# psy-ex/svt-av1-psy

Measured on AMD Instinct MI355X. Metric: Mblocks/s per kernel (SAD, FwdTxfm2d, CDEF) + encoder fps @1080p preset 8, higher is better.
Workload: dtype u8

## Files before the change

svt-av1-psy_amd/csrc/sad.hip:

```cpp
#include "svt_hip_common.h"
#include "../../include/svtav1_hip.h"
#include "hme_geom.h"
#include <vector>

namespace {

struct __attribute__((packed, aligned(4))) U64A4 { unsigned long long v; };
struct __attribute__((aligned(4))) u32x4_a4 { uint32_t x, y, z, w; };
struct __attribute__((aligned(16))) u32x4_a16 { uint32_t x, y, z, w; };

constexpr uint32_t MAX_SAD_VALUE = 128 * 128 * 255;
constexpr int      ME_TW         = 64;
constexpr int      ME_TH         = 32;
constexpr int      KEY_POS_BITS  = 11;
constexpr uint32_t ME_WAVE_MAX_W = 24, ME_WAVE_MAX_H = 16;

__device__ __forceinline__ void stage_rows_u8(uint32_t* lds, int pitch_dw, const uint8_t* g, uint32_t gstride, int width,
                                              int rows, int tid, int nthreads) {
    const int total = rows * pitch_dw;
    for (int i = tid; i < total; i += nthreads) {
        const int r   = i / pitch_dw;
        const int k   = i - r * pitch_dw;
        const int col = k * 4;
        uint32_t  v   = 0;
// ... 115 lines not shown
__device__ __forceinline__ uint32_t dpp_add_quad_xor2(uint32_t v) {
    return v + (uint32_t)__builtin_amdgcn_update_dpp(0, (int)v, 0x4E, 0xf, 0xf, false);
}
__device__ __forceinline__ uint32_t dpp_add_row_ror4(uint32_t v) {
    return v + (uint32_t)__builtin_amdgcn_update_dpp(0, (int)v, 0x124, 0xf, 0xf, false);
}
__device__ __forceinline__ uint32_t dpp_add_row_ror8(uint32_t v) {
    return v + (uint32_t)__builtin_amdgcn_update_dpp(0, (int)v, 0x128, 0xf, 0xf, false);
}
__device__ __forceinline__ uint32_t umin32(uint32_t a, uint32_t b) { return a < b ? a : b; }


constexpr int ME_PITCH = 34;

__device__ __forceinline__ uint32_t dpp_scatter_sum_quads(const uint32_t (&v)[4]) {
#ifdef SVT_HIP_EMU
    const uint32_t a0 = dpp_add_row_ror8(v[0]), a1 = dpp_add_row_ror8(v[1]), a2 = dpp_add_row_ror8(v[2]), a3 = dpp_add_row_ror8(v[3]);
    const uint32_t t0 = (uint32_t)__builtin_amdgcn_update_dpp((int)a0, (int)a2, 0xE4, 0xf, 0xc, false);
    const uint32_t t1 = (uint32_t)__builtin_amdgcn_update_dpp((int)a1, (int)a3, 0xE4, 0xf, 0xc, false);
    const uint32_t y  = (uint32_t)__builtin_amdgcn_update_dpp((int)t0, (int)t1, 0xE4, 0xf, 0xa, false);
    const uint32_t x  = y + (uint32_t)__builtin_amdgcn_update_dpp(0, (int)t0, 0x12C, 0xf, 0x5, false);
    return x + (uint32_t)__builtin_amdgcn_update_dpp(0, (int)t1, 0x124, 0xf, 0xa, false);
#else
    uint32_t t0, t1;
    asm("s_nop 1\n\t"
        "v_add_u32_dpp %0, %2, %2 row_ror:8 row_mask:0xf bank_mask:0x3\n\t"
        "v_add_u32_dpp %0, %4, %4 row_ror:8 row_mask:0xf bank_mask:0xc\n\t"
        "v_add_u32_dpp %1, %3, %3 row_ror:8 row_mask:0xf bank_mask:0x3\n\t"
        "v_add_u32_dpp %1, %5, %5 row_ror:8 row_mask:0xf bank_mask:0xc\n\t"
        "v_add_u32_dpp %0, %0, %0 row_ror:12 row_mask:0xf bank_mask:0x5\n\t"
        "s_nop 0\n\t"
        "v_add_u32_dpp %0, %1, %1 row_ror:4 row_mask:0xf bank_mask:0xa"
        : "=&v"(t0), "=&v"(t1)
        : "v"(v[0]), "v"(v[1]), "v"(v[2]), "v"(v[3]));
    return t0;
#endif
}

constexpr int ME_WAVE_QSUM_DW = 32;
__device__ __forceinline__ void me_lds_order() {
    __builtin_amdgcn_fence(__ATOMIC_ACQ_REL, "wavefront");
    __builtin_amdgcn_wave_barrier();
}
__device__ __forceinline__ uint32_t sum_rows_pair(const uint32_t a, const uint32_t b) {
#ifdef SVT_HIP_EMU
    const int l = (int)(threadIdx.x & 63);
    uint32_t  t = 0;
    for (int r = 0; r < 4; r++) {
        const uint32_t ar = (uint32_t)__shfl((int)a, (l & 15) + 16 * r), br = (uint32_t)__shfl((int)b, (l & 15) + 16 * r);
        t += ((l >> 4) & 1) ? br : ar;
    }
    return t;
#else
    const auto     x16 = __builtin_amdgcn_permlane16_swap(a, b, false, false);
    const uint32_t two = x16[0] + x16[1];
    const auto     x32 = __builtin_amdgcn_permlane32_swap(two, two, false, false);
    return x32[0] + x32[1];
#endif
}
template <bool SUB, bool FULL, int PITCH = ME_PITCH, bool QLDS = false>
__device__ __forceinline__ void me_search_strips(const uint32_t* __restrict__ win, const uint32_t (&s)[8][2], int Wt, int Ht, int g0, int gstep, int l,
                                                 uint32_t& best8, uint32_t& best16, uint32_t& best32, uint32_t& best64, unsigned long long* qsum = nullptr) {
    const int bx = (l & 1) | ((l >> 1) & 2) | ((l >> 2) & 4);
    const int by = ((l >> 1) & 1) | ((l >> 2) & 2) | ((l >> 3) & 4);
    const int q  = l & 3, c = (l >> 2) & 3;
    unsigned long long* const qslot = QLDS ? qsum + (l >> 2) : nullptr;
    const uint16_t* const     qmine = QLDS ? (const uint16_t*)qslot + q : nullptr;
    const int      G    = (Wt + 3) >> 2;
    const uint32_t qsel = 0x0c0c0100u + 0x0202u * (uint32_t)q;
    uint32_t       himask = 0xffff0000u;
    SVT_HIP_OPAQUE_I32(himask);
    constexpr uint32_t NO_STEP = 0x1ffffu;
    uint32_t       b16 = 0xffffffffu, b32 = 0xffffffffu, b64 = 0xffffffffu;
    constexpr bool PAIRG = QLDS && !SUB;
    uint32_t       b64s  = 0xffffffffu;
    constexpr uint32_t NO_SUM = 0x7ffffu;
    uint32_t       p32 = NO_SUM, b32p = 0xffffffffu, b64p = 0xffffffffu;
    int            kc = 0;
    for (int g = g0; g < G; g += gstep) {
        const uint32_t* colp   = win + (by * 8) * PITCH + bx * 2 + g;
        const int       nvalid = (Wt - 4 * g) < 4 ? (Wt - 4 * g) : 4;
        const uint32_t inv1 = nvalid > 1 ? 0u : 0xffffffffu, inv2 = nvalid > 2 ? 0u : 0xffffffffu, inv3 = nvalid > 3 ? 0u : 0xffffffffu;
        const uint32_t invq = q < nvalid ? 0u : 0xffffffffu;
        auto track16 = [&](const uint32_t sad16, const uint32_t at) {
            const uint32_t k16 = (sad16 << KEY_POS_BITS) | at;
            b16 = umin32(b16, FULL ? k16 : (k16 | invq));
        };
        auto track16x2 = [&](const uint32_t sad16a, const uint32_t sad16b, const uint32_t at) {
            const uint32_t ka = (sad16a << KEY_POS_BITS) | at, kb = (sad16b << KEY_POS_BITS) | (at + ME_TW);
            b16 = FULL ? umin32(umin32(b16, ka), kb) : umin32(b16, umin32(ka, kb) | invq);
        };
        U64A4 ra[8], rb[8];
#pragma unroll
        for (int r = 0; r < 7; r++) {
            ra[r] = *(const U64A4*)(colp + r * PITCH);
            rb[r] = *(const U64A4*)(colp + r * PITCH + 1);
        }
        uint32_t pos = (uint32_t)(4 * g);
        uint32_t v0  = 0;
        uint32_t s32a = 0;
        for (int yb = 0; yb < Ht; yb += 8) {
            const uint32_t* rowp = colp + (yb + 7) * PITCH;
#pragma unroll
            for (int h = 0; h < 2; h++) {
                if (yb + 4 * h < Ht) {
                    uint32_t v[4] = {NO_STEP, NO_STEP, NO_STEP, NO_STEP};
#pragma unroll
                    for (int j = 0; j < 4; j++) {
                        const int i = 4 * h + j;
                        if (yb + i < Ht) {
                            ra[(i + 7) & 7] = *(const U64A4*)(rowp + i * PITCH);
                            rb[(i + 7) & 7] = *(const U64A4*)(rowp + i * PITCH + 1);
                            unsigned long long acc = 0;
#pragma unroll
                            for (int r = 0; r < 8; r += (SUB ? 2 : 1)) {
                                acc = __builtin_amdgcn_qsad_pk_u16_u8(ra[(i + r) & 7].v, s[r][0], acc);
                                acc = __builtin_amdgcn_qsad_pk_u16_u8(rb[(i + r) & 7].v, s[r][1], acc);
                            }
                            if (SUB) acc <<= 1;
                            const uint32_t lo = (uint32_t)acc, hi = (uint32_t)(acc >> 32);
                            const uint32_t p1 = FULL ? pos + 1 : ((pos + 1) | inv1), p2 = FULL ? pos + 2 : ((pos + 2) | inv2), p3 = FULL ? pos + 3 : ((pos + 3) | inv3);
                            const uint32_t k0 = (lo << 16) | pos, k1 = (lo & himask) | p1, k2 = (hi << 16) | p2, k3 = (hi & himask) | p3;
                            best8 = umin32(umin32(best8, k0), k1);
                            best8 = umin32(umin32(best8, k2), k3);
                            if (QLDS) {
                                me_lds_order();
                                *qslot = 0ull;
                                me_lds_order();
                                atomicAdd(qslot, acc);
                                me_lds_order();
                                v[j] = *qmine;
                                if (PAIRG) {
                                    if (j == 2) track16x2(v[0], v[1], pos - 2 * ME_TW);
                                } else if (j > 0) {
                                    track16(v[j - 1], pos - ME_TW);
                                }
                            } else {
                                const uint32_t tlo = dpp_add_quad_xor2(dpp_add_quad_xor1(lo));
                                const uint32_t thi = dpp_add_quad_xor2(dpp_add_quad_xor1(hi));
                                v[j] = __builtin_amdgcn_perm(thi, tlo, qsel);
                                track16(v[j], pos);
                            }
                            pos += ME_TW;
                        }
                    }
                    if (PAIRG) {
                        const int left = Ht - (yb + 4 * h);
                        if (left >= 4) {
                            asm volatile("");
                            track16x2(v[2], v[3], pos - 2 * ME_TW);
                        } else if (left == 3) {
                            asm volatile("");
                            track16(v[2], pos - ME_TW);
                        } else if (left == 2) {
                            asm volatile("");
                            track16x2(v[0], v[1], pos - 2 * ME_TW);
                        } else {
                            track16(v[0], pos - ME_TW);
                        }
                    } else if (QLDS) {
                        const int left = Ht - (yb + 4 * h);
                        track16(left >= 4 ? v[3] : (left == 3 ? v[2] : (left == 2 ? v[1] : v[0])), pos - ME_TW);
                    }
                    v0 = v[0];
                    if (PAIRG) {
                        const int      left   = Ht - (yb + 4 * h);
                        const bool     paired = left >= 6 - 4 * h;
                        const uint32_t gposa  = (uint32_t)(4 * g + ME_TW * yb);
                        if (h == 0 && left >= 2) {
                            s32a = dpp_scatter_sum_quads(v);
                            if (!paired) {
                                const uint32_t k32 = (s32a << KEY_POS_BITS) | gposa;
                                b32 = umin32(b32, FULL ? k32 : (k32 | invq));
                                const uint32_t k64 = (sum_rows_pair(s32a, s32a) << KEY_POS_BITS) | gposa;
                                b64s = umin32(b64s, FULL ? k64 : (k64 | invq));
                            }
                        }
                        if (h == 1 && paired) {
                            const uint32_t s32b = dpp_scatter_sum_quads(v);
                            const uint32_t k32a = (s32a << KEY_POS_BITS) | gposa, k32b = (s32b << KEY_POS_BITS) | (gposa + 4 * ME_TW);
                            b32 = FULL ? umin32(umin32(b32, k32a), k32b) : umin32(b32, umin32(k32a, k32b) | invq);
                            const uint32_t k64 = (sum_rows_pair(s32a, s32b) << KEY_POS_BITS) | gposa;
                            b64 = umin32(b64, FULL ? k64 : (k64 | invq));
                        }
                    } else if (yb + 4 * h + 1 < Ht) {
                        const uint32_t gpos  = (uint32_t)(4 * g + ME_TW * (yb + 4 * h));
                        const uint32_t sad32 = dpp_scatter_sum_quads(v);
                        const uint32_t k32   = (sad32 << KEY_POS_BITS) | gpos;
                        b32 = umin32(b32, FULL ? k32 : (k32 | invq));
                        const auto     x16   = __builtin_amdgcn_permlane16_swap(sad32, sad32, false, false);
                        const uint32_t pair  = x16[0] + x16[1];
                        const auto     x32   = __builtin_amdgcn_permlane32_swap(pair, pair, false, false);
                        const uint32_t sad64 = x32[0] + x32[1];
                        const uint32_t k64   = (sad64 << KEY_POS_BITS) | gpos;
                        b64 = umin32(b64, FULL ? k64 : (k64 | invq));
                    }
                }
            }
        }
        if ((Ht & 3) == 1) {
            const uint32_t sum = dpp_add_row_ror4(dpp_add_row_ror8(v0));
            if (c == kc && (FULL || q < nvalid)) p32 = sum;
            if (++kc == 4 || g + gstep >= G) {
                const uint32_t gpos  = (uint32_t)(4 * (g - (kc - 1) * gstep) + ME_TW * (Ht - 1));
                b32p = umin32(b32p, (p32 << KEY_POS_BITS) | gpos);
                const auto     x16   = __builtin_amdgcn_permlane16_swap(p32, p32, false, false);
                const uint32_t pair  = x16[0] + x16[1];
                const auto     x32   = __builtin_amdgcn_permlane32_swap(pair, pair, false, false);
                const uint32_t sad64 = x32[0] + x32[1];
                b64p = umin32(b64p, (sad64 << KEY_POS_BITS) | gpos);
                p32 = NO_SUM;
                kc  = 0;
            }
        }
    }
    best16 = umin32(best16, b16 | (uint32_t)q);
    best32 = umin32(best32, b32 | (uint32_t)(q | (c << 6)));
    best64 = umin32(best64, b64 | (uint32_t)(q | (c << 6) | (PAIRG ? ((l << 4) & 256) : 0)));
    if (PAIRG) best64 = umin32(best64, b64s | (uint32_t)(q | (c << 6)));
    best32 = umin32(best32, b32p | (uint32_t)(q | (4 * gstep * c)));
    best64 = umin32(best64, b64p | (uint32_t)(q | (4 * gstep * c)));
}

template <bool SUB>
__global__ __launch_bounds__(256, 4) void me_fullpel_kernel(const uint8_t* __restrict__ src_base, const uint8_t* __restrict__ ref_base,
                                                         const SvtHipMeSearchDesc* __restrict__ descs, uint32_t n,
                                                         uint32_t tiles_x,
                                                         uint32_t* __restrict__ best_sad, uint32_t* __restrict__ best_mv,
                                                         unsigned long long* __restrict__ keys) {
    HIP_DYNAMIC_SHARED(uint32_t, smem)
    uint32_t* src_lds  = smem;
    uint32_t* best_lds = smem + 64 * 16;
    uint32_t* win      = smem + 64 * 16 + 88;

    const int      tid  = threadIdx.x;
    const uint32_t item = xcd_remap(blockIdx.x, n);
    const uint32_t tile = blockIdx.y;
    const SvtHipMeSearchDesc d = descs[item];
    const int W   = d.search_area_width, H = d.search_area_height;
    const int tx0 = (int)(tile % tiles_x) * ME_TW;
    const int ty0 = (int)(tile / tiles_x) * ME_TH;
    if (tx0 >= W || ty0 >= H) {
        if (tile == 0 && keys == nullptr && tid < SVT_HIP_ME_NUM_BLOCKS) {
            best_sad[(size_t)item * SVT_HIP_ME_NUM_BLOCKS + tid] = MAX_SAD_VALUE;
            best_mv[(size_t)item * SVT_HIP_ME_NUM_BLOCKS + tid]  = 0;
        }
        return;
    }
    const int Wt = (W - tx0) < ME_TW ? (W - tx0) : ME_TW;
    const int Ht = (H - ty0) < ME_TH ? (H - ty0) : ME_TH;

    {
        uint32_t vs[1][4], vw[3][4];
        stage_rows_load<1, 2>(vs, src_base + d.src_off, d.src_stride, 64, 64, tid);
        stage_rows_load<3, 3>(vw, ref_base + d.ref_off + (size_t)ty0 * d.ref_stride + tx0, d.ref_stride, 64 + Wt - 1, 64 + Ht - 1, tid);
        stage_rows_store<1, 2>(vs, src_lds, 16, 64, tid);
        stage_rows_store<3, 3>(vw, win, ME_PITCH, 64 + Ht - 1, tid);
    }
    if (tid < 88) best_lds[tid] = 0xffffffffu;
    __syncthreads();

    const int l  = tid & 63;
    const int wv = tid >> 6;
    uint32_t s[8][2];
    {
        const int bx = (l & 1) | ((l >> 1) & 2) | ((l >> 2) & 4);
        const int by = ((l >> 1) & 1) | ((l >> 2) & 2) | ((l >> 3) & 4);
#pragma unroll
        for (int r = 0; r < 8; r++) {
            s[r][0] = src_lds[(by * 8 + r) * 16 + bx * 2 + 0];
            s[r][1] = src_lds[(by * 8 + r) * 16 + bx * 2 + 1];
        }
    }
    uint32_t best8 = 0xffffffffu, best16 = 0xffffffffu, best32 = 0xffffffffu, best64 = 0xffffffffu;
    if ((Wt & 3) == 0) me_search_strips<SUB, true>(win, s, Wt, Ht, wv, 4, l, best8, best16, best32, best64);
    else me_search_strips<SUB, false>(win, s, Wt, Ht, wv, 4, l, best8, best16, best32, best64);

    atomicMin(&best_lds[21 + l], best8);
    atomicMin(&best_lds[5 + (l >> 2)], best16);
    atomicMin(&best_lds[1 + (l >> 4)], best32);
    atomicMin(&best_lds[0], best64);
    __syncthreads();
    if (tid < SVT_HIP_ME_NUM_BLOCKS) {
        const uint32_t key = best_lds[tid];
        const uint32_t sad = tid >= 21 ? (key >> 16) : (key >> KEY_POS_BITS);
        const int      X   = tx0 + (int)(key & 63u);
        const int      Y   = ty0 + (int)((key >> 6) & 31u);
        const size_t   o   = (size_t)item * SVT_HIP_ME_NUM_BLOCKS + tid;
        if (keys == nullptr) {
            best_sad[o] = sad;
            best_mv[o]  = ((uint32_t)(uint16_t)(Y + d.y_search_area_origin) << 16) | (uint16_t)(X + d.x_search_area_origin);
        } else {
            atomicMin(&keys[o], ((unsigned long long)sad << 32) | (unsigned long long)(uint32_t)(Y * W + X));
        }
    }
}

struct __attribute__((packed, aligned(1))) u32x2_a1 { uint32_t x, y; };
__device__ __forceinline__ uint32_t dpp_min_quad_xor1(uint32_t v) { return umin32(v, (uint32_t)__builtin_amdgcn_update_dpp(-1, (int)v, 0xB1, 0xf, 0xf, false)); }
__device__ __forceinline__ uint32_t dpp_min_quad_xor2(uint32_t v) { return umin32(v, (uint32_t)__builtin_amdgcn_update_dpp(-1, (int)v, 0x4E, 0xf, 0xf, false)); }
__device__ __forceinline__ uint32_t dpp_min_row_ror4(uint32_t v) { return umin32(v, (uint32_t)__builtin_amdgcn_update_dpp(-1, (int)v, 0x124, 0xf, 0xf, false)); }
__device__ __forceinline__ uint32_t dpp_min_row_ror8(uint32_t v) { return umin32(v, (uint32_t)__builtin_amdgcn_update_dpp(-1, (int)v, 0x128, 0xf, 0xf, false)); }

template <int NF, int PITCH>
__device__ __forceinline__ void stage_window_wave(uint32_t* lds, const uint8_t* g, const uint32_t gstride, const int width, const int rows, const int l) {
    constexpr int RPI = 64 / NF;
    const int     rem = width & 15, back = 16 - rem;
    const bool    p0 = rem != 0 && l < rows, p1 = rem != 0 && l + 64 < rows;
    u32x4_a1      t[2] = {{0u, 0u, 0u, 0u}, {0u, 0u, 0u, 0u}};
    const uint32_t tail_off = (uint32_t)l * gstride + (uint32_t)(width - 16);
    if (p0) t[0] = *(const u32x4_a1*)(g + tail_off);
    if (p1) t[1] = *(const u32x4_a1*)(g + (size_t)64 * gstride + tail_off);

    const int lr = l / NF, lc = l - lr * NF;
    if (lr < RPI) {
        const uint32_t goff = (uint32_t)lr * gstride + (uint32_t)lc * 16u;
        uint32_t*      lp   = lds + lr * PITCH + lc * 4;
        for (int r0 = 0; r0 < rows; r0 += 4 * RPI) {
            const uint8_t* gb = g + (size_t)r0 * gstride;
            u32x4_a1       v[4];
#pragma unroll
            for (int k = 0; k < 4; k++)
                if (r0 + k * RPI + lr < rows) v[k] = *(const u32x4_a1*)(gb + (size_t)(k * RPI) * gstride + goff);
#pragma unroll
            for (int k = 0; k < 4; k++)
                if (r0 + k * RPI + lr < rows) {
                    uint32_t* o = lp + (r0 + k * RPI) * PITCH;
                    *(u32x2_a8*)(o + 0) = u32x2_a8{v[k].x, v[k].y};
                    *(u32x2_a8*)(o + 2) = u32x2_a8{v[k].z, v[k].w};
                }
        }
    }
#pragma unroll
    for (int k = 0; k < 2; k++)
        if (k == 0 ? p0 : p1) {
            uint32_t x0 = t[k].x, x1 = t[k].y, x2 = t[k].z, x3 = t[k].w;
            if (back & 4) { x0 = x1; x1 = x2; x2 = x3; x3 = 0; }
            if (back & 8) { x0 = x2; x1 = x3; x2 = 0; x3 = 0; }
            const uint32_t bs = (uint32_t)back & 3u;
            x0 = __builtin_amdgcn_alignbyte(x1, x0, bs);
            x1 = __builtin_amdgcn_alignbyte(x2, x1, bs);
            x2 = __builtin_amdgcn_alignbyte(x3, x2, bs);
            x3 = __builtin_amdgcn_alignbyte(0u, x3, bs);
            uint32_t* o = lds + (l + 64 * k) * PITCH + NF * 4;
            if (NF * 4 + 0 < PITCH) *(u32x2_a8*)(o + 0) = u32x2_a8{x0, x1};
            if (NF * 4 + 2 < PITCH) *(u32x2_a8*)(o + 2) = u32x2_a8{x2, x3};
        }
}

template <bool SUB, int PITCH>
__global__ __launch_bounds__(256) void me_fullpel_wave_kernel(const uint8_t* __restrict__ src_base, const uint8_t* __restrict__ ref_base,
                                                              const SvtHipMeSearchDesc* __restrict__ descs, const uint32_t n, const int win_dw,
                                                              uint32_t* __restrict__ best_sad, uint32_t* __restrict__ best_mv) {
    HIP_DYNAMIC_SHARED(uint32_t, smem)
    const int      l    = threadIdx.x & 63, wv = __builtin_amdgcn_readfirstlane((int)(threadIdx.x >> 6));
    const uint32_t item = xcd_remap(blockIdx.x, gridDim.x) * 4 + (uint32_t)wv;
    if (item >= n) return;
    const SvtHipMeSearchDesc d = descs[item];
    const int    W = d.search_area_width, H = d.search_area_height;
    const size_t o = (size_t)item * SVT_HIP_ME_NUM_BLOCKS;
    if (W <= 0 || H <= 0) {
        for (int k = l; k < SVT_HIP_ME_NUM_BLOCKS; k += 64) { best_sad[o + k] = MAX_SAD_VALUE; best_mv[o + k] = 0; }
        return;
    }
    uint32_t* win = smem + wv * (win_dw + ME_WAVE_QSUM_DW);
    const int bx = (l & 1) | ((l >> 1) & 2) | ((l >> 2) & 4);
    const int by = ((l >> 1) & 1) | ((l >> 2) & 2) | ((l >> 3) & 4);
    uint32_t  s[8][2];
    {
        const uint8_t* sp = src_base + d.src_off + (size_t)(by * 8) * d.src_stride + bx * 8;
#pragma unroll
        for (int r = 0; r < 8; r++) {
            const u32x2_a1 t = *(const u32x2_a1*)(sp + (size_t)r * d.src_stride);
            s[r][0] = t.x; s[r][1] = t.y;
        }
    }
    const int width = 64 + W - 1;
    if (PITCH >= 22 && (width >> 4) == 5) stage_window_wave<5, PITCH>(win, ref_base + d.ref_off, d.ref_stride, width, 64 + H - 1, l);
    else stage_window_wave<4, PITCH>(win, ref_base + d.ref_off, d.ref_stride, width, 64 + H - 1, l);
    __builtin_amdgcn_wave_barrier();

    uint32_t best8 = 0xffffffffu, best16 = 0xffffffffu, best32 = 0xffffffffu, best64 = 0xffffffffu;
    if ((W & 3) == 0) me_search_strips<SUB, true, PITCH, true>(win, s, W, H, 0, 1, l, best8, best16, best32, best64, (unsigned long long*)(win + win_dw));
    else me_search_strips<SUB, false, PITCH, true>(win, s, W, H, 0, 1, l, best8, best16, best32, best64, (unsigned long long*)(win + win_dw));
    best16 = dpp_min_quad_xor2(dpp_min_quad_xor1(best16));
    best32 = dpp_min_row_ror8(dpp_min_row_ror4(dpp_min_quad_xor2(dpp_min_quad_xor1(best32))));
    best64 = dpp_min_row_ror8(dpp_min_row_ror4(dpp_min_quad_xor2(dpp_min_quad_xor1(best64))));
    {
        const auto x16 = __builtin_amdgcn_permlane16_swap(best64, best64, false, false);
        best64         = umin32(x16[0], x16[1]);
        const auto x32 = __builtin_amdgcn_permlane32_swap(best64, best64, false, false);
        best64         = umin32(x32[0], x32[1]);
    }
    const int xo = d.x_search_area_origin, yo = d.y_search_area_origin;
    auto emit = [&](const int idx, const uint32_t key, const bool is8) {
        const uint32_t sad = is8 ? (key >> 16) : (key >> KEY_POS_BITS);
        const int      X = (int)(key & 63u), Y = (int)((key >> 6) & 31u);
        best_sad[o + idx] = sad;
        best_mv[o + idx]  = ((uint32_t)(uint16_t)(Y + yo) << 16) | (uint16_t)(X + xo);
    };
    emit(21 + l, best8, true);
    const int      q    = l & 3;
    const uint32_t mine = q == 1 ? best16 : (q == 2 ? best32 : best64);
    const int      r32  = 64 * l - 56, r16 = 16 * l - 76;
    const uint32_t key  = (uint32_t)__builtin_amdgcn_ds_bpermute(l < 5 ? (r32 > 0 ? r32 : 0) : r16, (int)mine);
    if (l < 21) emit(l, key, false);
}

__global__ void me_finalize_kernel(const SvtHipMeSearchDesc* __restrict__ descs, uint32_t n, const unsigned long long* __restrict__ keys,
                                   uint32_t* __restrict__ best_sad, uint32_t* __restrict__ best_mv) {
    const uint32_t i = blockIdx.x * blockDim.x + threadIdx.x;
    if (i >= n * SVT_HIP_ME_NUM_BLOCKS) return;
    const SvtHipMeSearchDesc d   = descs[i / SVT_HIP_ME_NUM_BLOCKS];
    const unsigned long long key = keys[i];
    if (key == ~0ull) {
        best_sad[i] = MAX_SAD_VALUE;
        best_mv[i]  = 0;
        return;
    }
    const uint32_t pos = (uint32_t)key;
    const int      W   = d.search_area_width;
    const int      X = (int)(pos % (uint32_t)W), Y = (int)(pos / (uint32_t)W);
    best_sad[i]        = (uint32_t)(key >> 32);
    best_mv[i]         = ((uint32_t)(uint16_t)(Y + d.y_search_area_origin) << 16) | (uint16_t)(X + d.x_search_area_origin);
}

__device__ __forceinline__ uint32_t wave_sum(uint32_t v) {
    v += (uint32_t)__shfl_xor((int)v, 32);
    v += (uint32_t)__shfl_xor((int)v, 16);
    v = dpp_add_row_ror8(v);
    v = dpp_add_row_ror4(v);
    v = dpp_add_quad_xor2(v);
    v = dpp_add_quad_xor1(v);
    return v;
}

template <int CHUNK>
__device__ __forceinline__ uint32_t sad_chunks(const uint8_t* __restrict__ src, const uint8_t* __restrict__ ref, uint32_t ss, uint32_t rs,
                                               int cpr, int cshift, int total, int l) {
    uint32_t sad = 0;
    for (int i0 = l; i0 < total; i0 += 256) {
        uint32_t av[4][CHUNK / 4], bv[4][CHUNK / 4];
#pragma unroll
        for (int k = 0; k < 4; ++k) {
            const int  i  = i0 + 64 * k;
            const bool in = i < total;
            const int  r  = cshift >= 0 ? (i >> cshift) : (i / cpr);
            const int  c  = i - r * cpr;
            const uint8_t* pa = src + (size_t)r * ss + c * CHUNK;
            const uint8_t* pb = ref + (size_t)r * rs + c * CHUNK;
            if (CHUNK == 16) {
                u32x4_a1 a = {0, 0, 0, 0}, b = {0, 0, 0, 0};
                if (in) { a = *(const u32x4_a1*)pa; b = *(const u32x4_a1*)pb; }
                av[k][0] = a.x; av[k][CHUNK / 4 > 1 ? 1 : 0] = a.y; av[k][CHUNK / 4 > 2 ? 2 : 0] = a.z; av[k][CHUNK / 4 > 3 ? 3 : 0] = a.w;
                bv[k][0] = b.x; bv[k][CHUNK / 4 > 1 ? 1 : 0] = b.y; bv[k][CHUNK / 4 > 2 ? 2 : 0] = b.z; bv[k][CHUNK / 4 > 3 ? 3 : 0] = b.w;
            } else {
                u32_a1 a = {0}, b = {0};
                if (in) { a = *(const u32_a1*)pa; b = *(const u32_a1*)pb; }
                av[k][0] = a.x; bv[k][0] = b.x;
            }
        }
#pragma unroll
        for (int k = 0; k < 4; ++k)
#pragma unroll
            for (int j = 0; j < CHUNK / 4; ++j) sad = __builtin_amdgcn_sad_u8(av[k][j], bv[k][j], sad);
    }
    return sad;
}

__global__ __launch_bounds__(256) void sad_nxm_kernel(const uint8_t* __restrict__ src_base, const uint8_t* __restrict__ ref_base,
                                                      const SvtHipSadPair* __restrict__ pairs, uint32_t n, int width, int height,
                                                      uint32_t* __restrict__ sad_out) {
    const int      l    = threadIdx.x & 63;
    const uint32_t pair = xcd_remap(blockIdx.x, gridDim.x) * 4 + (threadIdx.x >> 6);
    if (pair >= n) return;
    const SvtHipSadPair p   = pairs[pair];
    const uint8_t*      src = src_base + p.src_off;
    const uint8_t*      ref = ref_base + p.ref_off;
    uint32_t            sad = 0;
    if ((width & 15) == 0) {
        const int cpr = width >> 4;
        sad = sad_chunks<16>(src, ref, p.src_stride, p.ref_stride, cpr, (cpr & (cpr - 1)) ? -1 : __builtin_ctz(cpr), cpr * height, l);
    } else if ((width & 3) == 0) {
        const int cpr = width >> 2;
        sad = sad_chunks<4>(src, ref, p.src_stride, p.ref_stride, cpr, (cpr & (cpr - 1)) ? -1 : __builtin_ctz(cpr), cpr * height, l);
    } else {
        const int total = width * height;
        for (int i = l; i < total; i += 64) {
            const int r = i / width, c = i - r * width;
            const int a = src[(size_t)r * p.src_stride + c], b = ref[(size_t)r * p.ref_stride + c];
            sad += (uint32_t)(a > b ? a - b : b - a);
        }
    }
    sad = wave_sum(sad);
    if (l == 0) sad_out[pair] = sad;
}

constexpr int SADP_PPW = 4;
struct SadRegs { uint32_t a[4][4], b[4][4]; };
__device__ __forceinline__ void sadp_issue(SadRegs& r, const uint8_t* __restrict__ src, const uint8_t* __restrict__ ref, const SvtHipSadPair& p, const int cpr,
                                           const int cshift, const int total, const int l) {
#pragma unroll
    for (int k = 0; k < 4; ++k) {
        const int  i  = l + 64 * k;
        const bool in = i < total;
        const int  rr = i >> cshift, c = i - (rr << cshift);
        u32x4_a1 a = {0, 0, 0, 0}, b = {0, 0, 0, 0};
        if (in) {
            a = *(const u32x4_a1*)(src + p.src_off + (size_t)rr * p.src_stride + c * 16);
            b = *(const u32x4_a1*)(ref + p.ref_off + (size_t)rr * p.ref_stride + c * 16);
        }
        r.a[k][0] = a.x; r.a[k][1] = a.y; r.a[k][2] = a.z; r.a[k][3] = a.w;
        r.b[k][0] = b.x; r.b[k][1] = b.y; r.b[k][2] = b.z; r.b[k][3] = b.w;
    }
}
__device__ __forceinline__ uint32_t sadp_reduce(const SadRegs& r) {
    uint32_t sad = 0;
#pragma unroll
    for (int k = 0; k < 4; ++k)
#pragma unroll
        for (int j = 0; j < 4; ++j) sad = __builtin_amdgcn_sad_u8(r.a[k][j], r.b[k][j], sad);
    return wave_sum(sad);
}
__global__ __launch_bounds__(256) void sad_nxm_pipe_kernel(const uint8_t* __restrict__ src_base, const uint8_t* __restrict__ ref_base,
                                                           const SvtHipSadPair* __restrict__ pairs, uint32_t n, int cshift , int total,
                                                           uint32_t* __restrict__ sad_out) {
    const int      l     = threadIdx.x & 63, w = __builtin_amdgcn_readfirstlane(threadIdx.x >> 6);
    const uint32_t first = xcd_remap(blockIdx.x, gridDim.x) * (4 * SADP_PPW) + (uint32_t)w;
    if (first >= n) return;
    const int cpr = 1 << cshift;
    SadRegs   cur, nxt;
    sadp_issue(cur, src_base, ref_base, pairs[first], cpr, cshift, total, l);
#pragma unroll
    for (int k = 0; k < SADP_PPW; ++k) {
        const uint32_t pair = first + 4u * (uint32_t)k, np = pair + 4u;
        const bool     more = k + 1 < SADP_PPW && np < n;
        if (more) sadp_issue(nxt, src_base, ref_base, pairs[np], cpr, cshift, total, l);
        const uint32_t sad = sadp_reduce(cur);
        if (l == 0) sad_out[pair] = sad;
        if (!more) break;
        cur = nxt;
    }
}

constexpr int SADS_SPW = 4;
struct StripRegs { uint32_t a[4][4], b[4][4]; };
__device__ __forceinline__ void strip_issue(StripRegs& r, const uint8_t* __restrict__ sp, const uint8_t* __restrict__ rp, const uint32_t ss, const uint32_t rs,
                                            const int row0, const int ro, const int height, const bool live) {
#pragma unroll
    for (int k = 0; k < 4; ++k) {
        const int row = row0 + 4 * k;
        u32x4_a1  a = {0, 0, 0, 0}, b = {0, 0, 0, 0};
        if (live && row + ro < height) {
            a = *(const u32x4_a1*)(sp + (size_t)row * ss);
            b = *(const u32x4_a1*)(rp + (size_t)row * rs);
        }
        r.a[k][0] = a.x; r.a[k][1] = a.y; r.a[k][2] = a.z; r.a[k][3] = a.w;
        r.b[k][0] = b.x; r.b[k][1] = b.y; r.b[k][2] = b.z; r.b[k][3] = b.w;
    }
}
__device__ __forceinline__ uint32_t strip_consume(const StripRegs& r, uint32_t sad) {
#pragma unroll
    for (int k = 0; k < 4; ++k)
#pragma unroll
        for (int j = 0; j < 4; ++j) sad = __builtin_amdgcn_sad_u8(r.a[k][j], r.b[k][j], sad);
    return sad;
}
__global__ __launch_bounds__(256) void sad_nxm_strip_kernel(const uint8_t* __restrict__ src_base, const uint8_t* __restrict__ ref_base,
                                                            const SvtHipSadPair* __restrict__ pairs, const uint32_t n, const int cshift ,
                                                            const int height, uint32_t* __restrict__ sad_out) {
    const int      l = threadIdx.x & 63, w = __builtin_amdgcn_readfirstlane(threadIdx.x >> 6);
    const int      cpr = 1 << cshift, nb = 16 >> cshift;
    const int      sb = (l & 15) >> cshift, j = l & (cpr - 1), ro = l >> 4;
    const int      groups = (height + 15) >> 4;
    const uint32_t strip0 = (xcd_remap(blockIdx.x, gridDim.x) * 4 + (uint32_t)w) * SADS_SPW;
    if (strip0 * (uint32_t)nb >= n) return;
    const uint8_t *sp = nullptr, *rp = nullptr;
    uint32_t       ss = 0, rs = 0;
    bool           live = false;
    auto open_strip = [&](const int k) {
        const uint32_t pair = (strip0 + (uint32_t)k) * (uint32_t)nb + (uint32_t)sb;
        live = k < SADS_SPW && pair < n;
        if (live) {
            const SvtHipSadPair p = pairs[pair];
            sp = src_base + p.src_off + (size_t)ro * p.src_stride + j * 16;
            rp = ref_base + p.ref_off + (size_t)ro * p.ref_stride + j * 16;
            ss = p.src_stride; rs = p.ref_stride;
        }
    };
    StripRegs cur, nxt;
    open_strip(0);
    strip_issue(cur, sp, rp, ss, rs, 0, ro, height, live);
    for (int k = 0; k < SADS_SPW; ++k) {
        if ((strip0 + (uint32_t)k) * (uint32_t)nb >= n) break;
        const bool     mine = live;
        uint32_t       sad  = 0;
        const uint32_t out  = (strip0 + (uint32_t)k) * (uint32_t)nb + (uint32_t)sb;
        for (int g = 0; g < groups; ++g) {
            if (g + 1 < groups) {
                strip_issue(nxt, sp, rp, ss, rs, 16 * (g + 1), ro, height, live);
            } else {
                open_strip(k + 1);
                strip_issue(nxt, sp, rp, ss, rs, 0, ro, height, live);
            }
            sad = strip_consume(cur, sad);
            cur = nxt;
        }
        for (int m = 1; m < cpr; m <<= 1) sad += (uint32_t)__shfl_xor((int)sad, m);
        sad += (uint32_t)__shfl_xor((int)sad, 16);
        sad += (uint32_t)__shfl_xor((int)sad, 32);
        if (mine && j == 0 && ro == 0) sad_out[out] = sad;
    }
}

__global__ __launch_bounds__(64) void sad_16b_kernel(const uint16_t* __restrict__ src, uint32_t src_stride, const uint16_t* __restrict__ ref,
                                                     uint32_t ref_stride, int width, int height, uint32_t* __restrict__ out) {
    const int l     = threadIdx.x;
    uint32_t  sad   = 0;
    const int total = width * height;
    for (int i = l; i < total; i += 64) {
        const int r = i / width, c = i - r * width;
        const int a = src[(size_t)r * src_stride + c], b = ref[(size_t)r * ref_stride + c];
        sad += (uint32_t)(a > b ? a - b : b - a);
    }
    sad = wave_sum(sad);
    if (l == 0) out[0] = sad;
}

template <int LXG>
__device__ __forceinline__ void sad_loop_item(uint32_t* smem, unsigned long long& wg_best, const uint8_t* __restrict__ src_base,
                                              const uint8_t* __restrict__ ref_base, const SvtHipSadLoopDesc& d, const uint32_t item, const uint32_t tile,
                                              const uint32_t tiles_x, unsigned long long* __restrict__ keys) {
    constexpr int TW = 4 << LXG, TH = 256 >> LXG;
    const int tid = threadIdx.x;
    const int W = d.search_area_width, H = d.search_area_height;
    const int bw = d.block_width, bh = d.block_height;
    const int tx0 = (int)(tile % tiles_x) * TW, ty0 = (int)(tile / tiles_x) * TH;
    if (tx0 >= W || ty0 >= H) return;
    const int Wt = (W - tx0) < TW ? (W - tx0) : TW;
    const int Ht = (H - ty0) < TH ? (H - ty0) : TH;
    const int src_pitch = ((bw + 15) >> 4) << 2;
    const int win_w     = bw + Wt - 1;
    const int win_pitch = (((bw + TW + 3) >> 2) + 3) & ~1;
    uint32_t* src_lds   = smem;
    uint32_t* win       = smem + src_pitch * bh;
    stage_rows_u8(src_lds, src_pitch, src_base + d.src_off, d.src_stride, bw, bh, tid, 256);
    if (tid == 0) wg_best = ~0ull;
    const int rstep    = (int)(d.ref_stride / d.src_stride_raw);
    const int win_rows = Ht + rstep * (bh - 1);
    const uint8_t* wsrc = ref_base + d.ref_off + (size_t)ty0 * d.src_stride_raw + tx0;
    if (win_w >= 16) stage_rows_wide_any(win, win_pitch, wsrc, d.src_stride_raw, win_w, win_rows, tid);
    else stage_rows_u8(win, win_pitch, wsrc, d.src_stride_raw, win_w, win_rows, tid, 256);
    __syncthreads();

    const int gx = tid & ((1 << LXG) - 1), yy = tid >> LXG;
    const bool skip_rule = (bw == 16) && (bh <= 16) && d.skip_search_line;
    unsigned long long best = ~0ull;
    if (yy < Ht && 4 * gx < Wt && !(skip_rule && (((ty0 + yy) & 1) == 0))) {
        uint32_t sad[4] = {0, 0, 0, 0};
        const int full_dw = bw >> 2, tail = bw & 3;
        for (int y = 0; y < bh; y++) {
            const uint32_t* rrow = win + (yy + rstep * y) * win_pitch + gx;
            const uint32_t* srow = src_lds + y * src_pitch;
            unsigned long long acc = 0;
            uint32_t prev = rrow[0];
            int      k    = 0;
            for (; k + 4 <= full_dw; k += 4) {
                const u32x4_a16 sv = *(const u32x4_a16*)(srow + k);
                const U64A4     n0 = *(const U64A4*)(rrow + k + 1), n1 = *(const U64A4*)(rrow + k + 3);
                const uint32_t  r1 = (uint32_t)n0.v, r2 = (uint32_t)(n0.v >> 32), r3 = (uint32_t)n1.v, r4 = (uint32_t)(n1.v >> 32);
                acc  = __builtin_amdgcn_qsad_pk_u16_u8(((unsigned long long)r1 << 32) | prev, sv.x, acc);
                acc  = __builtin_amdgcn_qsad_pk_u16_u8(n0.v, sv.y, acc);
                acc  = __builtin_amdgcn_qsad_pk_u16_u8(((unsigned long long)r3 << 32) | r2, sv.z, acc);
                acc  = __builtin_amdgcn_qsad_pk_u16_u8(n1.v, sv.w, acc);
                prev = r4;
                if ((k & 12) == 12) {
                    sad[0] += (uint32_t)acc & 0xffffu; sad[1] += (uint32_t)(acc >> 16) & 0xffffu;
                    sad[2] += (uint32_t)(acc >> 32) & 0xffffu; sad[3] += (uint32_t)(acc >> 48);
                    acc = 0;
                }
            }
            for (; k < full_dw; k++) {
                const uint32_t next = rrow[k + 1];
                acc  = __builtin_amdgcn_qsad_pk_u16_u8(((unsigned long long)next << 32) | prev, srow[k], acc);
                prev = next;
            }
            sad[0] += (uint32_t)acc & 0xffffu; sad[1] += (uint32_t)(acc >> 16) & 0xffffu;
            sad[2] += (uint32_t)(acc >> 32) & 0xffffu; sad[3] += (uint32_t)(acc >> 48);
            if (tail) {
                const uint32_t mask = (1u << (8 * tail)) - 1u;
                const uint32_t next = rrow[full_dw + 1];
                const uint32_t sv   = srow[full_dw] & mask;
#pragma unroll
                for (int j = 0; j < 4; j++) {
                    const uint32_t rv = __builtin_amdgcn_alignbyte(next, prev, (uint32_t)j) & mask;
                    sad[j]            = __builtin_amdgcn_sad_u8(rv, sv, sad[j]);
                }
// ... 975 lines not shown
```

Baseline: 28390.

## Unroll ME window staging with clamped rows and force scalar descriptor/base registers

Rewrites the per-wave search-window staging so each lane issues all its global loads up front as a fully unrolled batch, clamping out-of-range rows to the last row instead of predicating them, then writes to LDS afterwards. Adds inline-asm hints that keep base pointers, kernel arguments and the descriptor words in scalar registers so loads use SGPR base plus a VGPR lane offset. The aim is more memory-level parallelism, fewer branches and less VGPR address arithmetic. The cost is more registers per lane for the in-flight loads, redundant loads and LDS writes for the clamped rows, and a dependence on the descriptor layout staying fixed.

```diff
diff --git a/svt-av1-psy_amd/csrc/sad.hip b/svt-av1-psy_amd/csrc/sad.hip
--- a/svt-av1-psy_amd/csrc/sad.hip
+++ b/svt-av1-psy_amd/csrc/sad.hip
@@ -441,38 +441,58 @@
 __device__ __forceinline__ uint32_t dpp_min_row_ror4(uint32_t v) { return umin32(v, (uint32_t)__builtin_amdgcn_update_dpp(-1, (int)v, 0x124, 0xf, 0xf, false)); }
 __device__ __forceinline__ uint32_t dpp_min_row_ror8(uint32_t v) { return umin32(v, (uint32_t)__builtin_amdgcn_update_dpp(-1, (int)v, 0x128, 0xf, 0xf, false)); }
 
+#ifdef SVT_HIP_EMU
+#define ME_SCALARS_HERE(x, ...) ((void)0)
+#else
+#define ME_SCALARS_HERE(x, ...) asm("" : "+s"(x) : __VA_ARGS__)
+#endif
+template <typename T>
+__device__ __forceinline__ T me_load_at(const uint8_t* base, const uint32_t lane_off) {
+#ifdef SVT_HIP_EMU
+    return *(const T*)(base + lane_off);
+#else
+    typedef uint32_t __attribute__((ext_vector_type(sizeof(T) / 4))) vec_t;
+    typedef vec_t __attribute__((aligned(1))) vec_a1_t;
+    static_assert(sizeof(T) == sizeof(vec_t), "dwords");
+    uintptr_t b = (uintptr_t)base;
+    asm("" : "+s"(b));
+    const vec_t x = *(const __attribute__((address_space(1))) vec_a1_t*)(b + (uintptr_t)lane_off);
+    T           t;
+    __builtin_memcpy(&t, &x, sizeof(T));
+    return t;
+#endif
+}
+
+constexpr int ME_WAVE_MAX_ROWS = 64 + (int)ME_WAVE_MAX_H - 1;
 template <int NF, int PITCH>
 __device__ __forceinline__ void stage_window_wave(uint32_t* lds, const uint8_t* g, const uint32_t gstride, const int width, const int rows, const int l) {
     constexpr int RPI = 64 / NF;
-    const int     rem = width & 15, back = 16 - rem;
-    const bool    p0 = rem != 0 && l < rows, p1 = rem != 0 && l + 64 < rows;
-    u32x4_a1      t[2] = {{0u, 0u, 0u, 0u}, {0u, 0u, 0u, 0u}};
-    const uint32_t tail_off = (uint32_t)l * gstride + (uint32_t)(width - 16);
-    if (p0) t[0] = *(const u32x4_a1*)(g + tail_off);
-    if (p1) t[1] = *(const u32x4_a1*)(g + (size_t)64 * gstride + tail_off);
-
-    const int lr = l / NF, lc = l - lr * NF;
-    if (lr < RPI) {
-        const uint32_t goff = (uint32_t)lr * gstride + (uint32_t)lc * 16u;
-        uint32_t*      lp   = lds + lr * PITCH + lc * 4;
-        for (int r0 = 0; r0 < rows; r0 += 4 * RPI) {
-            const uint8_t* gb = g + (size_t)r0 * gstride;
-            u32x4_a1       v[4];
-#pragma unroll
-            for (int k = 0; k < 4; k++)
-                if (r0 + k * RPI + lr < rows) v[k] = *(const u32x4_a1*)(gb + (size_t)(k * RPI) * gstride + goff);
-#pragma unroll
-            for (int k = 0; k < 4; k++)
-                if (r0 + k * RPI + lr < rows) {
-                    uint32_t* o = lp + (r0 + k * RPI) * PITCH;
-                    *(u32x2_a8*)(o + 0) = u32x2_a8{v[k].x, v[k].y};
-                    *(u32x2_a8*)(o + 2) = u32x2_a8{v[k].z, v[k].w};
-                }
-        }
-    }
-#pragma unroll
-    for (int k = 0; k < 2; k++)
-        if (k == 0 ? p0 : p1) {
+    constexpr int NP  = (ME_WAVE_MAX_ROWS + RPI - 1) / RPI;
+    constexpr int NPF = 64 / RPI;
+    const int      rem = width & 15, back = 16 - rem;
+    const uint32_t last = (uint32_t)(rows - 1);
+    const uint32_t tr1  = umin32((uint32_t)l + 64u, last);
+    u32x4_a1       t[2], v[NP];
+    t[0] = me_load_at<u32x4_a1>(g, (uint32_t)l * gstride + (uint32_t)(width - 16));
+    t[1] = me_load_at<u32x4_a1>(g, tr1 * gstride + (uint32_t)(width - 16));
+
+    const int      le = (NF * RPI < 64 && l >= NF * RPI) ? l - NF : l;
+    const int      lr = le / NF, lc = le - lr * NF;
+    const uint32_t goff = (uint32_t)lr * gstride + (uint32_t)lc * 16u;
+    uint32_t*      lp   = lds + lr * PITCH + lc * 4;
+    uint32_t       rk[NP];
+#pragma unroll
+    for (int k = 0; k < NP; k++) {
+        if (k < NPF) {
+            v[k] = me_load_at<u32x4_a1>(g + (size_t)(k * RPI) * gstride, goff);
+        } else {
+            rk[k] = umin32((uint32_t)(lr + k * RPI), last);
+            v[k]  = me_load_at<u32x4_a1>(g, rk[k] * gstride + (uint32_t)lc * 16u);
+        }
+    }
+    if (rem != 0) {
+#pragma unroll
+        for (int k = 0; k < 2; k++) {
             uint32_t x0 = t[k].x, x1 = t[k].y, x2 = t[k].z, x3 = t[k].w;
             if (back & 4) { x0 = x1; x1 = x2; x2 = x3; x3 = 0; }
             if (back & 8) { x0 = x2; x1 = x3; x2 = 0; x3 = 0; }
@@ -481,11 +501,21 @@
             x1 = __builtin_amdgcn_alignbyte(x2, x1, bs);
             x2 = __builtin_amdgcn_alignbyte(x3, x2, bs);
             x3 = __builtin_amdgcn_alignbyte(0u, x3, bs);
-            uint32_t* o = lds + (l + 64 * k) * PITCH + NF * 4;
+            uint32_t* o = lds + (k == 0 ? (uint32_t)l : tr1) * PITCH + NF * 4;
             if (NF * 4 + 0 < PITCH) *(u32x2_a8*)(o + 0) = u32x2_a8{x0, x1};
             if (NF * 4 + 2 < PITCH) *(u32x2_a8*)(o + 2) = u32x2_a8{x2, x3};
         }
-}
+    }
+#pragma unroll
+    for (int k = 0; k < NP; k++) {
+        uint32_t* o = k < NPF ? lp + (k * RPI) * PITCH : lds + rk[k] * PITCH + lc * 4;
+        *(u32x2_a8*)(o + 0) = u32x2_a8{v[k].x, v[k].y};
+        *(u32x2_a8*)(o + 2) = u32x2_a8{v[k].z, v[k].w};
+    }
+}
+
+struct __attribute__((aligned(8))) MeDescWords { uint32_t w[8]; };
+static_assert(sizeof(SvtHipMeSearchDesc) == 32, "descriptor layout");
 
 template <bool SUB, int PITCH>
 __global__ __launch_bounds__(256) void me_fullpel_wave_kernel(const uint8_t* __restrict__ src_base, const uint8_t* __restrict__ ref_base,
@@ -493,10 +523,16 @@
                                                               uint32_t* __restrict__ best_sad, uint32_t* __restrict__ best_mv) {
     HIP_DYNAMIC_SHARED(uint32_t, smem)
     const int      l    = threadIdx.x & 63, wv = __builtin_amdgcn_readfirstlane((int)(threadIdx.x >> 6));
+    uint32_t nn = n;
+    ME_SCALARS_HERE(nn, "s"(src_base), "s"(ref_base), "s"(descs), "s"(win_dw), "s"(best_sad), "s"(best_mv));
     const uint32_t item = xcd_remap(blockIdx.x, gridDim.x) * 4 + (uint32_t)wv;
-    if (item >= n) return;
-    const SvtHipMeSearchDesc d = descs[item];
-    const int    W = d.search_area_width, H = d.search_area_height;
+    if (item >= nn) return;
+    MeDescWords dw = *(const MeDescWords*)(descs + item);
+    ME_SCALARS_HERE(dw.w[7], "s"(dw.w[0]), "s"(dw.w[1]), "s"(dw.w[2]), "s"(dw.w[3]), "s"(dw.w[4]), "s"(dw.w[5]), "s"(dw.w[6]));
+    const size_t   src_off = (size_t)dw.w[0] | ((size_t)dw.w[1] << 32), ref_off = (size_t)dw.w[2] | ((size_t)dw.w[3] << 32);
+    const uint32_t src_stride = dw.w[4], ref_stride = dw.w[5];
+    const int      xo = (int16_t)(dw.w[6] & 0xffffu), yo = (int16_t)(dw.w[6] >> 16);
+    const int      W = (int)(dw.w[7] & 0xffffu), H = (int)(dw.w[7] >> 16);
     const size_t o = (size_t)item * SVT_HIP_ME_NUM_BLOCKS;
     if (W <= 0 || H <= 0) {
         for (int k = l; k < SVT_HIP_ME_NUM_BLOCKS; k += 64) { best_sad[o + k] = MAX_SAD_VALUE; best_mv[o + k] = 0; }
@@ -507,16 +543,17 @@
     const int by = ((l >> 1) & 1) | ((l >> 2) & 2) | ((l >> 3) & 4);
     uint32_t  s[8][2];
     {
-        const uint8_t* sp = src_base + d.src_off + (size_t)(by * 8) * d.src_stride + bx * 8;
+        const uint8_t* sp  = src_base + src_off;
+        const uint32_t slo = (uint32_t)(by * 8) * src_stride + (uint32_t)(bx * 8);
 #pragma unroll
         for (int r = 0; r < 8; r++) {
-            const u32x2_a1 t = *(const u32x2_a1*)(sp + (size_t)r * d.src_stride);
+            const u32x2_a1 t = me_load_at<u32x2_a1>(sp + (size_t)r * src_stride, slo);
             s[r][0] = t.x; s[r][1] = t.y;
         }
     }
     const int width = 64 + W - 1;
-    if (PITCH >= 22 && (width >> 4) == 5) stage_window_wave<5, PITCH>(win, ref_base + d.ref_off, d.ref_stride, width, 64 + H - 1, l);
-    else stage_window_wave<4, PITCH>(win, ref_base + d.ref_off, d.ref_stride, width, 64 + H - 1, l);
+    if (PITCH >= 22 && (width >> 4) == 5) stage_window_wave<5, PITCH>(win, ref_base + ref_off, ref_stride, width, 64 + H - 1, l);
+    else stage_window_wave<4, PITCH>(win, ref_base + ref_off, ref_stride, width, 64 + H - 1, l);
     __builtin_amdgcn_wave_barrier();
 
     uint32_t best8 = 0xffffffffu, best16 = 0xffffffffu, best32 = 0xffffffffu, best64 = 0xffffffffu;
@@ -531,7 +568,6 @@
         const auto x32 = __builtin_amdgcn_permlane32_swap(best64, best64, false, false);
         best64         = umin32(x32[0], x32[1]);
     }
-    const int xo = d.x_search_area_origin, yo = d.y_search_area_origin;
     auto emit = [&](const int idx, const uint32_t key, const bool is8) {
         const uint32_t sad = is8 ? (key >> 16) : (key >> KEY_POS_BITS);
         const int      X = (int)(key & 63u), Y = (int)((key >> 6) & 31u);
```

Result: faster. 28920 (median of 6 runs) (+1.9%).
